# RapidAI/RapidDoc

Hardware: AMD Instinct MI355X
Metric: pages/sec (layout+OCR det/rec) (higher is better)
Workload: dtype f32

## Files before the change

rapiddoc_amd/_lib.py:

```python
from __future__ import annotations

import ctypes as C
from pathlib import Path

_PKG = Path(__file__).resolve().parent
LIB_PATH = _PKG / "librapiddoc_mi355.so"
_lib = None

SYMBOLS = {
    "rd_version": (C.c_char_p, []),
    "rd_create": (C.c_void_p, [C.c_int, C.c_char_p]),
    "rd_create_error": (C.c_char_p, []),
    "rd_destroy": (None, [C.c_void_p]),
    "rd_last_error": (C.c_char_p, [C.c_void_p]),
    "rd_load_weights": (C.c_int, [C.c_void_p, C.c_void_p, C.c_size_t]),
    "rd_query_workspace": (C.c_int, [C.c_void_p, C.c_int, C.c_int, C.c_int, C.c_int, C.POINTER(C.c_size_t)]),
    "rd_det_forward": (C.c_int, [C.c_void_p, C.c_void_p, C.c_int, C.c_int, C.c_int, C.c_void_p, C.c_void_p, C.c_size_t, C.c_void_p]),
    "rd_det_forward_ex": (C.c_int, [C.c_void_p, C.c_void_p, C.c_int, C.c_int, C.c_int, C.c_void_p, C.c_int, C.c_void_p, C.c_void_p, C.c_size_t, C.c_void_p]),
    "rd_rec_forward": (C.c_int, [C.c_void_p, C.c_void_p, C.c_int, C.c_int, C.c_void_p, C.c_void_p, C.c_void_p, C.c_int, C.c_void_p, C.c_size_t, C.c_void_p]),
    "rd_rec_num_classes": (C.c_int, [C.c_void_p]),
    "rd_rec_token_dim": (C.c_int, [C.c_void_p]),
    "rd_rec_backbone_forward": (C.c_int, [C.c_void_p, C.c_void_p, C.c_int, C.c_int, C.c_void_p, C.c_void_p, C.c_size_t, C.c_void_p]),
    "rd_rec_backbone_forward_lines": (C.c_int, [C.c_void_p, C.c_void_p, C.c_int, C.c_int, C.c_void_p, C.c_void_p, C.c_void_p, C.c_size_t, C.c_void_p]),
    "rd_rec_tail_forward": (C.c_int, [C.c_void_p, C.c_void_p, C.c_int, C.c_int, C.c_int, C.c_void_p, C.c_void_p, C.c_void_p, C.c_void_p,
# ... 28 lines not shown
                                     C.c_int, C.c_void_p, C.c_size_t, C.c_void_p, C.c_int, C.c_void_p, C.c_void_p]),
    "rd_rec_chunk_cost": (C.c_double, [C.c_int, C.c_int, C.c_int]),
    "rd_rec_plan_chunks": (C.c_int, [C.c_void_p, C.c_int, C.c_int, C.c_int, C.c_int, C.c_int, C.c_void_p, C.c_int, C.c_void_p]),
    "rd_rec_plan_lines": (C.c_int, [C.c_void_p, C.c_void_p] + [C.c_int] * 9 + [C.c_void_p] * 4 + [C.c_int, C.c_void_p]),
    "rd_text_boxes_order_merge": (C.c_int, [C.c_void_p, C.c_void_p, C.c_int, C.c_int, C.c_void_p, C.c_void_p]),
    "rd_ctc_rows_text": (C.c_int, [C.c_void_p, C.c_int, C.c_int, C.c_void_p, C.c_int64, C.c_void_p, C.c_void_p, C.c_void_p, C.c_void_p]),
    "rd_layout_postprocess": (C.c_int, [C.c_void_p, C.c_int, C.c_int, C.c_int, C.c_int, C.c_void_p, C.c_void_p, C.c_void_p, C.c_void_p]),
    "rd_layout_postprocess_select": (C.c_int, [C.c_void_p, C.c_int, C.c_int, C.c_int, C.c_int, C.c_void_p, C.c_void_p, C.c_void_p, C.c_void_p]),
    "rd_find_external_contours": (C.c_int, [C.c_void_p, C.c_int, C.c_int, C.c_void_p, C.c_int, C.c_void_p, C.c_int, C.c_void_p, C.c_void_p]),
    "rd_find_external_contours_none": (C.c_int, [C.c_void_p, C.c_int, C.c_int, C.c_void_p, C.c_int, C.c_void_p, C.c_int, C.c_void_p, C.c_void_p]),
    "rd_checkbox_workspace": (C.c_size_t, [C.c_int, C.c_int, C.c_int, C.c_int, C.c_int, C.c_void_p]),
    "rd_checkbox_detect_device": (C.c_int, [C.c_int, C.c_void_p, C.c_int, C.c_int, C.c_int, C.c_int, C.c_int, C.c_int, C.c_void_p, C.c_size_t, C.c_void_p,
                                            C.c_void_p, C.c_void_p]),
    "rd_checkbox_finish": (C.c_int, [C.c_void_p, C.c_int, C.c_int, C.c_int, C.c_void_p, C.c_int, C.c_void_p]),
    "rd_region_canvases_workspace": (C.c_size_t, [C.c_int, C.c_int, C.c_int]),
    "rd_region_canvases": (C.c_int, [C.c_int, C.c_void_p, C.c_int, C.c_void_p, C.c_void_p, C.c_int, C.c_int, C.c_void_p, C.c_void_p, C.c_void_p, C.c_size_t,
                                     C.c_void_p]),
    "rd_contour_area": (C.c_double, [C.c_void_p, C.c_int]),
    "rd_arc_length": (C.c_double, [C.c_void_p, C.c_int, C.c_int]),
    "rd_approx_poly_dp": (C.c_int, [C.c_void_p, C.c_int, C.c_double, C.c_int, C.c_void_p, C.c_void_p]),
    "rd_min_area_rect_points": (C.c_int, [C.c_void_p, C.c_int, C.c_void_p]),
    "rd_polygon_area": (C.c_double, [C.c_void_p, C.c_int]),
    "rd_polygon_intersection_area": (C.c_double, [C.c_void_p, C.c_int, C.c_void_p, C.c_int]),
    "rd_fill_poly": (C.c_int, [C.c_void_p, C.c_int, C.c_int, C.c_void_p, C.c_int, C.c_int]),
    "rd_msdeform_attn": (C.c_int, [C.c_int] + [C.c_void_p] * 6 + [C.c_int] * 7 + [C.c_void_p]),
    "rd_topk_rows": (C.c_int, [C.c_int, C.c_void_p, C.c_int, C.c_int, C.c_int, C.c_void_p, C.c_void_p, C.c_void_p]),
    "rd_encoder_layer_workspace": (C.c_size_t, [C.c_int, C.c_int, C.c_int]),
    "rd_encoder_layer": (C.c_int, [C.c_int, C.c_void_p, C.c_void_p] + [C.c_int] * 6 + [C.c_void_p] * 12 + [C.c_float, C.c_void_p, C.c_void_p, C.c_size_t, C.c_void_p]),
    "rd_set_precision": (C.c_int, [C.c_void_p, C.c_char_p]),
    "rd_range_status": (C.c_int, [C.c_void_p, C.c_void_p]),
    "rd_plan_stats": (C.c_int, [C.c_void_p, C.POINTER(C.c_uint64), C.POINTER(C.c_uint64), C.POINTER(C.c_uint64)]),
    "rd_set_profiling": (C.c_int, [C.c_void_p, C.c_int]),
    "rd_profile_json": (C.c_char_p, [C.c_void_p]),
}

_I, _P, _F = C.c_int, C.c_void_p, C.c_float
DEBUG_SYMBOLS = {
    "rd_debug_det_forward_stages": (_I, [_P, _P, _I, _I, _I, _P, _P, _P]),
    "rd_debug_cls_forward_stages": (_I, [_P, _P, _I, _I, _I, _P, _P, _P, _P]),
    "rd_debug_table_decode": (_I, [_P, _P, _I, _I, _I, _P] + [_P] * 7),
    "rd_debug_table_decode_stream": (_I, [_P, _P, _I, _I, _I, _I, _P, _P, _P, _P, _P, _P, _P, _P, _I]),
    "rd_debug_table_encoder_taps": (_I, [_P, _P, _I, _I, _I, _P, _P, _P]),
    "rd_debug_formula_decode": (_I, [_P, _P, _I, _I, _I, _P, C.POINTER(C.c_int32), _P, _P, _P]),
    "rd_debug_formula_decode_stream": (_I, [_P, _P, _I, _I, _I, _I, _P, _P, _P, _P, _P, _P, _P, _I]),
    "rd_debug_resize_aa_coeffs": (_I, [_I, _I, _P, _P, C.c_int64]),
    "rd_debug_resample_coeffs": (_I, [_I, _I, C.c_double, C.c_double, _I, _P, _P, C.c_int64]),
    "rd_debug_region_keep_mask": (_I, [_I, _I, _P, _I, _P]),
    "rd_debug_time_mixer": (_F, [_I] * 4 + [_P] * 6),
    "rd_debug_time_gemm": (_F, [_I] * 5 + [_P] * 6),
    "rd_debug_gemm_h1": (_F, [_I] * 5 + [_P, _I, _P, _P, _P, _I, _P, _I, _P]),
    "rd_debug_seqconv": (_F, [_I] * 8 + [_P, _I, _P, _I, _P, _P, _P, _P, _I, _P]),
    "rd_debug_det_local": (_F, [_I] * 5 + [_P] * 5 + [_F, _P, C.POINTER(C.c_int)]),
    "rd_debug_conv_route": (_I, [_I] * 17 + [_P, _I]),
    "rd_debug_conv_ex": (_F, [_I] * 22 + [_P] * 10 + [C.c_char_p, _P, _I, _P]),
    "rd_debug_conv": (_F, [_I] * 14 + [_P] * 8),
    "rd_debug_stem34": (_F, [_I] * 11 + [_P] * 7),
    "rd_debug_dwconv_ex": (_F, [_I] * 17 + [_P] * 10 + [_I]),
    "rd_debug_dwconv": (_F, [_I] * 8 + [_P] * 8),
    "rd_debug_dw_route": (_I, [_I] * 9 + [_P, _I, _P]),
    "rd_debug_weight_split": (_I, [_P, _I, _I, _P, _P]),
    "rd_debug_lcv3_dw": (_F, [_I] * 9 + [_P] * 8),
    "rd_debug_dw5_strip": (_F, [_I] * 11 + [_P] * 7),
    "rd_debug_mv1e_pool": (_I, [_I] * 4 + [_P] * 3),
    "rd_debug_derived_tensor": (C.c_long, [C.c_char_p, C.c_char_p, C.c_size_t, C.c_char_p, _P, C.c_long]),
    "rd_debug_mbv3_dw": (_F, [_I] * 12 + [_P] * 4),
    "rd_debug_mbv3_block": (_F, [_I] * 14 + [_P] * 8),
    "rd_debug_mbv3_block_ok": (_I, [_I] * 12),
    "rd_debug_mbv3s_dw": (_F, [_I] * 13 + [_P] * 4),
    "rd_debug_mbv3s_block": (_F, [_I] * 15 + [_P] * 12),
    "rd_debug_lcv3_dw_det": (_F, [_I] * 10 + [_P] * 5),
    "rd_debug_lcv3_block": (_F, [_I] * 9 + [_P] * 9),
    "rd_debug_time_ctc": (_F, [_I] * 4 + [_P] * 7 + [_I, _P]),
    "rd_debug_time_checkbox_mask": (_F, [_I] * 4 + [_P, _P]),
    "rd_debug_attention": (_I, [_I] * 4 + [_F, _P, _P, _P, _I, _P]),
    "rd_debug_vit_attention": (_I, [_I] * 4 + [_F, _P, _P]),
    "rd_debug_attention_limits": (_I, [_I, _P, _P]),
    "rd_debug_layernorm": (_I, [_I, _I, _P, _I, _P, _I, _P, _P, _F]),
    "rd_debug_se_chain": (_I, [_I] * 7 + [_F] + [_I] * 3 + [_P] * 9),
    "rd_debug_maxpool2x2s1": (_I, [_I] * 6 + [_P] * 2),
    "rd_debug_avgpool3x2": (_I, [_I] * 6 + [_P] * 3),
    "rd_debug_mask_cols": (_I, [_I] * 5 + [_P, _P, _I]),
    "rd_debug_upsample": (_I, [_I] * 8 + [_P] * 2),
    "rd_debug_add": (_I, [_I] * 5 + [_P] * 3),
    "rd_debug_det_head_tail": (_I, [_I] * 4 + [_P] * 6),
    "rd_debug_ctc_head": (_I, [_I] * 3 + [_P, _I] + [_P] * 6 + [_I, _P, _P]),
    "rd_debug_dec_gemv": (_I, [_I] * 4 + [_P] * 7),
    "rd_debug_dec_attention": (_I, [_I] * 4 + [_P, _P, _I, C.c_longlong] + [_P] * 5 + [_P, _I, _P, _P, _I, _P, _I]),
    "rd_debug_dec_select": (_I, [_I, _P, _I, _I, _I, _P, _I, _P, _I, _I] + [_P] * 6),
}


class NativeLibraryError(RuntimeError):
    pass


def load():
    global _lib
    if _lib is not None:
        return _lib
    if not LIB_PATH.exists():
        raise NativeLibraryError(
            f"{LIB_PATH} is missing - build it with `python -m rapiddoc_amd.build` (hipcc, gfx950). "
            "rapiddoc_amd has no CPU fallback.")
    import torch
    lib = C.CDLL(str(LIB_PATH))
    for name, (res, args) in {**SYMBOLS, **DEBUG_SYMBOLS}.items():
        fn = getattr(lib, name)
        fn.restype = res
        fn.argtypes = args
    _lib = lib
    return lib
```

rapiddoc_amd/csrc/api_debug.cpp:

```cpp
#include <algorithm>
#include <cstring>
#include <functional>
#include <string>
#include <vector>

#include "api_handle.h"
#include "builder_util.h"
#include "region_geom.h"

extern "C" {

static float rd_debug_time(int iters, const std::function<void()>& launch, const std::function<void()>& after_first = nullptr) {
    hipEvent_t e0, e1;
    (void)hipEventCreate(&e0); (void)hipEventCreate(&e1);
    launch();
    if (after_first) after_first();
    (void)hipEventRecord(e0, nullptr);
    for (int i = 0; i < iters; ++i) launch();
    (void)hipEventRecord(e1, nullptr);
    (void)hipEventSynchronize(e1);
    float ms = 0.f;
    (void)hipEventElapsedTime(&ms, e0, e1);
    (void)hipEventDestroy(e0); (void)hipEventDestroy(e1);
    return iters > 0 ? ms / iters : 0.f;
// ... 763 lines not shown
    const bool ok = hipDeviceSynchronize() == hipSuccess && hipGetLastError() == hipSuccess;
    if (range_out) *range_out = flag ? (int)*flag : 0;
    if (flag) (void)hipHostFree(flag);
    return ok ? 0 : -1;
}

int rd_debug_attention(int B, int T, int heads, int hd, float scale, float* qkv, float* o, const int32_t* seg, int route, int* range_out) {
    if (range_out) *range_out = 0;
    if (B <= 0 || T <= 0 || heads <= 0 || !(hd == 15 || hd == 16 || hd == 32) || route < 0 || route > 2) return -1;
    if (route == 2 && !rd::attention_h3_applies(1, hd)) return -1;
    unsigned* flag = debug_flag_new();
    if (!flag) return -1;
    if (route == 0) rd::launch_attention(qkv, o, B, T, heads, hd, scale, nullptr, seg, flag);
    else if (route == 1) rd::launch_attention_valu(qkv, o, B, T, heads, hd, scale, nullptr, seg);
    else rd::launch_attention_h3(qkv, o, B, T, heads, hd, scale, nullptr, seg, flag);
    return debug_finish(flag, range_out);
}
int rd_debug_vit_attention(int B, int T, int heads, int hd, float scale, float* qkv, float* o) {
    if (B <= 0 || B > 65535 || heads <= 0 || heads > 65535 || !qkv || !o || !rd::vit_attention_applies(T, hd)) return -1;
    rd::launch_vit_attention(qkv, o, B, T, heads, scale, nullptr);
    return debug_finish(nullptr, nullptr);
}
int rd_debug_attention_limits(int hd, int* h3_max_t, int* valu_lds_keys) {
    if (!(hd == 15 || hd == 16 || hd == 32)) return -1;
    if (h3_max_t) *h3_max_t = rd::attention_h3_applies(1, hd) ? rd::attention_h3_max_t() : 0;
    if (valu_lds_keys) *valu_lds_keys = rd::attention_lds_keys(hd);
    return 0;
}

int rd_debug_layernorm(int M, int C, float* x, int xld, float* y, int yld, float* g, float* b, float eps) {
    if (M <= 0 || C <= 0 || xld < C || yld < C) return -1;
    if (C == 768) {
        if (xld % 4 || yld % 4) return -1;
        rd::launch_layernorm768(x, xld, y, yld, g, b, M, eps, nullptr);
        return debug_finish(nullptr, nullptr);
    }
    if (C > 512) return -1;
    rd::launch_layernorm(x, xld, y, yld, g, b, M, C, eps, nullptr);
    return debug_finish(nullptr, nullptr);
}

int rd_debug_se_chain(int N, int H, int W, int C, int Cr, int chunks, int gate_act, float alpha, int xld, int yld, int fill_partial, float* x,
                      float* w1, float* b1, float* w2, float* b2, const int32_t* line_w, float* partial, float* gate_out, float* y) {
    if (N <= 0 || H <= 0 || W <= 0 || !rd::se_fc_shape_ok(C) || Cr <= 0 || Cr > 4096 || chunks <= 0) return -1;
    if (!w1 || !b1 || !w2 || !b2 || !partial || !gate_out || (fill_partial && line_w)) return -1;
    if ((fill_partial || y) && (!x || xld < C || xld % 4 != 0)) return -1;
    if (y && (yld < C || yld % 4 != 0)) return -1;
    const int hw = H * W;
    if (fill_partial) rd::launch_gap_partial(x, xld, N, hw, C, partial, chunks, nullptr);
    rd::SeFcParams f{};
    f.partial = partial; f.chunks = chunks; f.N = N; f.C = C; f.Cr = Cr; f.inv_hw = 1.f / (float)hw;
    f.w1 = w1; f.b1 = b1; f.w2 = w2; f.b2 = b2; f.gate = gate_act; f.scale = gate_out; f.H = H;
    if (line_w) { f.line_w = line_w; f.line_w_stride = 1; }
    rd::launch_se_fc(f, nullptr);
    if (y) rd::launch_scale_channels(x, xld, y, yld, gate_out, alpha, N, hw, C, nullptr);
    return debug_finish(nullptr, nullptr);
}

int rd_debug_maxpool2x2s1(int N, int H, int W, int C, int xld, int yld, float* x, float* y) {
    if (N <= 0 || H <= 0 || W <= 0 || C <= 0 || C % 4 || !x || !y || xld < C || xld % 4 || yld < C || yld % 4) return -1;
    rd::launch_maxpool2x2s1(x, xld, y, yld, N, H, W, C, nullptr);
    return debug_finish(nullptr, nullptr);
}
int rd_debug_avgpool3x2(int N, int H, int W, int C, int xld, int yld, float* x, float* y, const int32_t* line_tab) {
    if (N <= 0 || H < 3 || W < 2 || C <= 0 || C % 4 || !x || !y || xld < C || xld % 4 || yld < C || yld % 4 || (line_tab && H / 3 != 1)) return -1;
    rd::launch_avgpool3x2(x, xld, y, yld, N, H, W, C, nullptr, line_tab);
    return debug_finish(nullptr, nullptr);
}
int rd_debug_mask_cols(int N, int H, int W, int C, int yld, float* y, const int32_t* line_w, int stride) {
    if (N <= 0 || H <= 0 || W <= 0 || C <= 0 || C % 4 || !y || yld < C || yld % 4 || !line_w || stride < 1) return -1;
    rd::launch_mask_cols(y, yld, N, H, W, C, line_w, stride, nullptr);
    return debug_finish(nullptr, nullptr);
}
int rd_debug_upsample(int N, int H, int W, int C, int f, int accumulate, int xld, int yld, float* x, float* y) {
    if (N <= 0 || H <= 0 || W <= 0 || C <= 0 || C % 4 || f < 1 || H % f || W % f || !x || !y || xld < C || xld % 4 || yld < C || yld % 4) return -1;
    rd::launch_upsample(x, xld, y, yld, N, H, W, C, f, accumulate, nullptr);
    return debug_finish(nullptr, nullptr);
}
int rd_debug_add(int M, int C, int ald, int bld, int yld, float* a, float* b, float* y) {
    if (M <= 0 || C <= 0 || C % 4 || !a || !b || !y || ald < C || ald % 4 || bld < C || bld % 4 || yld < C || yld % 4) return -1;
    rd::launch_add(a, ald, b, bld, y, yld, M, C, nullptr);
    return debug_finish(nullptr, nullptr);
}

int rd_debug_det_head_tail(int N, int H, int W, int xld, float* x, float* w1, float* b1, float* w2, float* b2, float* y) {
    constexpr int kC = 24;
    if (N <= 0 || H <= 0 || W <= 0 || !x || !w1 || !b1 || !w2 || !b2 || !y || xld < kC || xld % 4 || !rd::det_head_tail_supported(kC, kC, 1)) return -1;
    std::vector<float> h1((size_t)kC * kC * 4), hb1(kC), h2((size_t)kC * 4), hb2(1);
    if (hipMemcpy(h1.data(), w1, h1.size() * 4, hipMemcpyDeviceToHost) != hipSuccess || hipMemcpy(hb1.data(), b1, hb1.size() * 4, hipMemcpyDeviceToHost) != hipSuccess ||
        hipMemcpy(h2.data(), w2, h2.size() * 4, hipMemcpyDeviceToHost) != hipSuccess || hipMemcpy(hb2.data(), b2, 4, hipMemcpyDeviceToHost) != hipSuccess)
        return -1;
    const std::vector<float> one(kC, 1.f), zero(kC, 0.f);
    std::vector<float> wa, ba, wb;
    rd::pack_det_head_tail(h1.data(), hb1.data(), h2.data(), kC, kC, one.data(), zero.data(), wa, ba, wb);
    std::vector<float> img(wa);
    img.insert(img.end(), ba.begin(), ba.end());
    img.insert(img.end(), wb.begin(), wb.end());
    img.push_back(hb2[0]);
    float* d = nullptr;
    if (hipMalloc((void**)&d, img.size() * 4) != hipSuccess) return -1;
    (void)hipMemcpy(d, img.data(), img.size() * 4, hipMemcpyHostToDevice);
    rd::launch_det_head_tail(x, xld, N, H, W, d, d + wa.size(), d + wa.size() + ba.size(), d + wa.size() + ba.size() + wb.size(), y, nullptr);
    const int rc = debug_finish(nullptr, nullptr);
    (void)hipFree(d);
    return rc;
}

int rd_debug_ctc_head(int M, int K, int Ccls, float* x, int xld, float* wp, void* wh, void* wl, float* part, int32_t* idx, float* prob,
                      int nsplit_override, int* nsplit_out, int* range_out) {
    if (range_out) *range_out = 0;
    if (M <= 0 || Ccls <= 0 || K <= 0 || K >= 128 || K % 4 || xld < K || xld % 4 || nsplit_override > 64 || (wh == nullptr) != (wl == nullptr)) return -1;
    rd::CtcParams p{};
    p.x = x; p.xld = xld; p.w = wp; p.M = M; p.K = K; p.C = Ccls; p.part = part;
    p.nsplit = nsplit_override > 0 ? nsplit_override : rd::ctc_head_nsplit(M, Ccls, wh != nullptr);
    p.idx = idx; p.prob = prob;
    p.wh = (const uint16_t*)wh; p.wl = (const uint16_t*)wl;
    if (nsplit_out) *nsplit_out = p.nsplit;
    unsigned* flag = debug_flag_new();
    if (!flag) return -1;
    p.range_flag = flag;
    rd::launch_ctc_head(p, nullptr);
    return debug_finish(flag, range_out);
}

int rd_debug_dec_gemv(int M, int K, int N, int act, const float* x, const float* w, const float* bias, const float* ln_g, const float* ln_b,
                      const float* res, float* y) {
    return rd::debug_dec_gemv(M, K, N, act, x, w, bias, ln_g, ln_b, res, y);
}
int rd_debug_dec_attention(int route, int self, int B, int T, float* kc, float* vc, int ldkv, long long seq_stride, const float* x,
                           const float* ln_g, const float* ln_b, const float* w, const float* bias, const float* q, int ldq, const float* kcur,
                           const float* vcur, int ldcur, float* out, int ldo) {
    return rd::debug_dec_attention(route, self, B, T, kc, vc, ldkv, seq_stride, x, ln_g, ln_b, w, bias, q, ldq, kcur, vcur, ldcur, out, ldo);
}
int rd_debug_dec_select(int mode, const float* logits, int V, int B, int step, int64_t* ids, int ids_ld, int32_t* unfinished, int n_unfinished,
                        int max_new, const float* emb, const float* pos, const float* g, const float* b, float* x, int32_t* state_out) {
    return rd::debug_dec_select(mode, logits, V, B, step, reinterpret_cast<long long*>(ids), ids_ld, unfinished, n_unfinished, max_new, emb, pos, g,
                                b, x, state_out);
}

}
```

rapiddoc_amd/csrc/kernels_misc.hip:

```cpp
#include <cstdlib>
#include <stdexcept>
#include <string>

#include "rd_device.h"

namespace rd {


__device__ __forceinline__ f32x4 act4(f32x4 v, int act) {
    f32x4 r = {rd_act(v[0], act), rd_act(v[1], act), rd_act(v[2], act), rd_act(v[3], act)};
    return r;
}

static inline int grid_for(long total, int block = 256, int cap = 16384) {
    long g = (total + block - 1) / block;
    if (g < 1) g = 1;
    return (int)(g > cap ? cap : g);
}

__global__ void __launch_bounds__(256) dwconv_kernel(DwParams p) {
    const int c4n = p.C >> 2;
    const long total = (long)p.N * p.OH * p.OW * c4n;
    for (long idx = (long)blockIdx.x * 256 + threadIdx.x; idx < total; idx += (long)gridDim.x * 256) {
        const int c = (int)(idx % c4n) << 2;
// ... 538 lines not shown
}
bool det_head_tail_supported(int cin, int cmid, int cout) { return cin == 24 && cmid == 24 && cout == 1; }
void launch_det_head_tail(const float* x, int xld, int N, int H, int W, const float* w1, const float* b1, const float* w2, const float* b2,
                          float* y, hipStream_t s) {
    const long total = (long)N * H * W;
    hipLaunchKernelGGL((det_head_tail_kernel<24, 24>), dim3((unsigned)((total + 255) / 256)), dim3(256), 0, s, x, xld, N, H, W, w1, b1, w2,
                       b2, y);
}

__global__ void __launch_bounds__(256) upsample_kernel(const float* x, int xld, float* y, int yld, int H, int W, int C,
                                                       int f, int accumulate, long total) {
    const int c4n = C >> 2;
    const int IH = H / f, IW = W / f;
    for (long idx = (long)blockIdx.x * 256 + threadIdx.x; idx < total; idx += (long)gridDim.x * 256) {
        const int c = (int)(idx % c4n) << 2;
        const long pix = idx / c4n;
        const int w = pix % W;
        const int h = (pix / W) % H;
        const int n = pix / ((long)W * H);
        f32x4 v = *reinterpret_cast<const f32x4*>(x + (((size_t)n * IH + h / f) * IW + w / f) * xld + c);
        float* yp = y + (size_t)pix * yld + c;
        if (accumulate) v += *reinterpret_cast<const f32x4*>(yp);
        *reinterpret_cast<f32x4*>(yp) = v;
    }
}
void launch_upsample(const float* x, int xld, float* y, int yld, int N, int H, int W, int C, int f, int accumulate,
                     hipStream_t s) {
    const long total = (long)N * H * W * (C >> 2);
    hipLaunchKernelGGL(upsample_kernel, dim3(grid_for(total)), dim3(256), 0, s, x, xld, y, yld, H, W, C, f, accumulate,
                       total);
}

__global__ void __launch_bounds__(256) add_kernel(const float* a, int ald, const float* b, int bld, float* y, int yld,
                                                  int C, long total) {
    const int c4n = C >> 2;
    for (long idx = (long)blockIdx.x * 256 + threadIdx.x; idx < total; idx += (long)gridDim.x * 256) {
        const int c = (int)(idx % c4n) << 2;
        const long m = idx / c4n;
        const f32x4 v = *reinterpret_cast<const f32x4*>(a + (size_t)m * ald + c) +
                        *reinterpret_cast<const f32x4*>(b + (size_t)m * bld + c);
        *reinterpret_cast<f32x4*>(y + (size_t)m * yld + c) = v;
    }
}
void launch_add(const float* a, int ald, const float* b, int bld, float* y, int yld, int M, int C, hipStream_t s) {
    const long total = (long)M * (C >> 2);
    hipLaunchKernelGGL(add_kernel, dim3(grid_for(total)), dim3(256), 0, s, a, ald, b, bld, y, yld, C, total);
}

__device__ __forceinline__ float wave_sum(float v) {
#pragma unroll
    for (int o = 32; o > 0; o >>= 1) v += __shfl_xor(v, o, 64);
    return v;
}
__device__ __forceinline__ float wave_max(float v) {
#pragma unroll
    for (int o = 32; o > 0; o >>= 1) v = fmaxf(v, __shfl_xor(v, o, 64));
    return v;
}

__global__ void __launch_bounds__(256) layernorm_kernel(const float* x, int xld, float* y, int yld, const float* g,
                                                        const float* b, int M, int C, float eps) {
    const int lane = threadIdx.x & 63;
    const int row = blockIdx.x * 4 + (threadIdx.x >> 6);
    if (row >= M) return;
    const float* xr = x + (size_t)row * xld;
    float v[8];
    float s = 0.f;
    int cnt = 0;
    for (int c = lane; c < C; c += 64) {
        v[cnt] = xr[c];
        s += v[cnt++];
    }
    const float mean = wave_sum(s) / C;
    float q = 0.f;
    for (int i = 0; i < cnt; ++i) {
        const float d = v[i] - mean;
        q += d * d;
    }
    const float rstd = rsqrtf(wave_sum(q) / C + eps);
    float* yr = y + (size_t)row * yld;
    cnt = 0;
    for (int c = lane; c < C; c += 64) yr[c] = (v[cnt++] - mean) * rstd * g[c] + b[c];
}
void launch_layernorm(const float* x, int xld, float* y, int yld, const float* g, const float* b, int M, int C,
                      float eps, hipStream_t s) {
    hipLaunchKernelGGL(layernorm_kernel, dim3((M + 3) / 4), dim3(256), 0, s, x, xld, y, yld, g, b, M, C, eps);
}

template <int HD>
__global__ void __launch_bounds__(256) attention_kernel(const float* qkv, float* o, int T, int heads, float scale, const int32_t* seg,
                                                        int tk_cap, int skip_upto) {
    constexpr int HDP = (HD + 3) / 4 * 4;
    constexpr int NV = HDP / 4;
    extern __shared__ float sm[];
    const int TL = min(T, tk_cap);
    f32x4* Ks = reinterpret_cast<f32x4*>(sm);
    f32x4* Vs = Ks + (size_t)TL * NV;
    const int b = blockIdx.x, h = blockIdx.y;
    const int C = heads * HD;
    size_t tok0 = (size_t)b * T;
    if (seg) {
        tok0 = (size_t)seg[2 * b];
        T = seg[2 * b + 1];
        if (T <= skip_upto) return;
    }
    const float* base = qkv + tok0 * 3 * C;
    auto stage = [&](int k0, int kn, bool with_v) {
        for (int i = threadIdx.x; i < kn * HDP; i += 256) {
            const int t = i / HDP, d = i - t * HDP;
            reinterpret_cast<float*>(Ks)[i] = d < HD ? base[(size_t)(k0 + t) * 3 * C + C + h * HD + d] : 0.f;
            if (with_v) reinterpret_cast<float*>(Vs)[i] = d < HD ? base[(size_t)(k0 + t) * 3 * C + 2 * C + h * HD + d] : 0.f;
        }
    };
    const bool tiled = T > TL;
    if (!tiled) {
        stage(0, T, true);
        __syncthreads();
    }
    const int rounds = (T + 255) / 256;
    for (int r = 0; r < rounds; ++r) {
        const int t = r * 256 + threadIdx.x;
        const bool live = t < T;
        f32x4 q[NV];
        const float* qrow = base + (size_t)min(t, T - 1) * 3 * C + h * HD;
#pragma unroll
        for (int v = 0; v < NV; ++v)
#pragma unroll
            for (int e = 0; e < 4; ++e) q[v][e] = qrow[min(4 * v + e, HD - 1)];
#pragma unroll
        for (int v = 0; v < NV; ++v)
#pragma unroll
            for (int e = 0; e < 4; ++e) q[v][e] = (live && 4 * v + e < HD) ? q[v][e] * scale : 0.f;
        auto dot = [&](int j) {
            float sdot = 0.f;
#pragma unroll
            for (int v = 0; v < NV; ++v) {
                const f32x4 kv = Ks[(size_t)j * NV + v];
#pragma unroll
                for (int e = 0; e < 4; ++e)
                    if (4 * v + e < HD) sdot = fmaf(q[v][e], kv[e], sdot);
            }
            return sdot;
        };
        float mx = -INFINITY;
        if (!tiled) {
            if (live)
                for (int j = 0; j < T; ++j) mx = fmaxf(mx, dot(j));
        } else {
            for (int k0 = 0; k0 < T; k0 += TL) {
                const int kn = min(TL, T - k0);
                __syncthreads();
                stage(k0, kn, false);
                __syncthreads();
                if (live)
                    for (int j = 0; j < kn; ++j) mx = fmaxf(mx, dot(j));
            }
        }
        float l = 0.f;
        f32x4 acc[NV];
#pragma unroll
        for (int v = 0; v < NV; ++v) acc[v] = f32x4{0.f, 0.f, 0.f, 0.f};
        auto accumulate = [&](int kn) {
            for (int j0 = 0; j0 < kn; j0 += 64) {
                const int je = min(kn, j0 + 64);
                float lr = 0.f;
                f32x4 ar[NV];
#pragma unroll
                for (int v = 0; v < NV; ++v) ar[v] = f32x4{0.f, 0.f, 0.f, 0.f};
                for (int j = j0; j < je; ++j) {
// ... 77 lines not shown
    smx[threadIdx.x] = mx;
    smi[threadIdx.x] = mi;
    __syncthreads();
    for (int o = 128; o > 0; o >>= 1) {
        if (threadIdx.x < o) {
            const float a = smx[threadIdx.x], b = smx[threadIdx.x + o];
            const int ia = smi[threadIdx.x], ib = smi[threadIdx.x + o];
            if (b > a || (b == a && ib < ia)) { smx[threadIdx.x] = b; smi[threadIdx.x] = ib; }
        }
        __syncthreads();
    }
    const float gmx = smx[0];
    float s = 0.f;
    for (int c = threadIdx.x; c < C; c += 256) s += __expf(zr[c] - gmx);
    ssum[threadIdx.x] = s;
    __syncthreads();
    for (int o = 128; o > 0; o >>= 1) {
        if (threadIdx.x < o) ssum[threadIdx.x] += ssum[threadIdx.x + o];
        __syncthreads();
    }
    if (threadIdx.x == 0) {
        idx[row] = smi[0];
        prob[row] = 1.f / ssum[0];
    }
}
void launch_rowmax_softmax(const float* logits, int ld, int M, int C, int32_t* idx, float* prob, hipStream_t s) {
    if (M > 0) hipLaunchKernelGGL(rowmax_softmax_kernel, dim3(M), dim3(256), 0, s, logits, ld, M, C, idx, prob);
}

__global__ void __launch_bounds__(256) row_softmax_kernel(const float* z, int ld, float* out, int C, int32_t* idx, float* prob) {
    const int row = blockIdx.x;
    const float* zr = z + (size_t)row * ld;
    float mx = -INFINITY;
    for (int c = threadIdx.x; c < C; c += 256) mx = fmaxf(mx, zr[c]);
    __shared__ float red[4];
    mx = wave_max(mx);
    if ((threadIdx.x & 63) == 0) red[threadIdx.x >> 6] = mx;
    __syncthreads();
    mx = fmaxf(fmaxf(red[0], red[1]), fmaxf(red[2], red[3]));
    __syncthreads();
    float s = 0.f;
    for (int c = threadIdx.x; c < C; c += 256) s += __expf(zr[c] - mx);
    s = wave_sum(s);
    if ((threadIdx.x & 63) == 0) red[threadIdx.x >> 6] = s;
    __syncthreads();
    const float inv = 1.f / (red[0] + red[1] + red[2] + red[3]);
    float* orow = out + (size_t)row * C;
    int first = 0x7fffffff;
    for (int c = threadIdx.x; c < C; c += 256) {
        const float pv = __expf(zr[c] - mx) * inv;
        orow[c] = pv;
        if (pv == inv && c < first) first = c;
    }
    if (idx == nullptr) return;
#pragma unroll
    for (int o = 32; o > 0; o >>= 1) first = min(first, __shfl_xor(first, o, 64));
    __shared__ int redi[4];
    if ((threadIdx.x & 63) == 0) redi[threadIdx.x >> 6] = first;
    __syncthreads();
    if (threadIdx.x == 0) {
        idx[row] = min(min(redi[0], redi[1]), min(redi[2], redi[3]));
        prob[row] = inv;
    }
}
void launch_row_softmax(const float* logits, int ld, float* out, int M, int C, hipStream_t s, int32_t* idx, float* prob) {
    if (M > 0) hipLaunchKernelGGL(row_softmax_kernel, dim3(M), dim3(256), 0, s, logits, ld, out, C, idx, prob);
}

__global__ void __launch_bounds__(256) nhwc_to_nchw_kernel(const float* x, int xld, float* y, int HW, int C) {
    __shared__ float tile[32][33];
    const int n = blockIdx.z;
    const int p0 = blockIdx.x * 32, c0 = blockIdx.y * 32;
    const int tx = threadIdx.x & 31, ty = threadIdx.x >> 5;
    for (int r = ty; r < 32; r += 8) {
        const int pp = p0 + r, c = c0 + tx;
        tile[r][tx] = (pp < HW && c < C) ? x[((size_t)n * HW + pp) * xld + c] : 0.f;
    }
    __syncthreads();
    for (int r = ty; r < 32; r += 8) {
        const int c = c0 + r, pp = p0 + tx;
        if (c < C && pp < HW) y[((size_t)n * C + c) * HW + pp] = tile[tx][r];
    }
}
void launch_nhwc_to_nchw(const float* x, int xld, float* y, int N, int H, int W, int C, hipStream_t s) {
    const int HW = H * W;
    hipLaunchKernelGGL(nhwc_to_nchw_kernel, dim3((HW + 31) / 32, (C + 31) / 32, N), dim3(256), 0, s, x, xld, y, HW, C);
}
__global__ void __launch_bounds__(256) nchw_to_nhwc_kernel(const float* x, float* y, int yld, int HW, int C) {
    __shared__ float tile[32][33];
    const int n = blockIdx.z;
    const int p0 = blockIdx.x * 32, c0 = blockIdx.y * 32;
    const int tx = threadIdx.x & 31, ty = threadIdx.x >> 5;
    for (int r = ty; r < 32; r += 8) {
        const int c = c0 + r, pp = p0 + tx;
        tile[r][tx] = (pp < HW && c < C) ? x[((size_t)n * C + c) * HW + pp] : 0.f;
    }
    __syncthreads();
    for (int r = ty; r < 32; r += 8) {
        const int pp = p0 + r, c = c0 + tx;
        if (c < C && pp < HW) y[((size_t)n * HW + pp) * yld + c] = tile[tx][r];
    }
}
void launch_nchw_to_nhwc(const float* x, float* y, int yld, int N, int C, int H, int W, hipStream_t s) {
    const int HW = H * W;
    hipLaunchKernelGGL(nchw_to_nhwc_kernel, dim3((HW + 31) / 32, (C + 31) / 32, N), dim3(256), 0, s, x, y, yld, HW, C);
}

__global__ void __launch_bounds__(256) crop_batch_kernel(CropBatchParams p) {
    const int i = blockIdx.y;
    const CropDesc d = p.descs[i];
    const long plane = (long)p.OH * p.OWp;
    float* dst = p.dst + (size_t)i * 3 * plane;
    const uint8_t* src = p.pages + (size_t)d.page * p.page_stride;
    const float sx = d.rot90 ? d.crop_h / d.out_w : d.crop_w / d.out_w;
    const float sy = d.rot90 ? d.crop_w / p.OH : d.crop_h / p.OH;
    for (long idx = (long)blockIdx.x * 256 + threadIdx.x; idx < plane; idx += (long)gridDim.x * 256) {
        const int ox = idx % p.OWp, oy = idx / p.OWp;
        float out[3] = {0.f, 0.f, 0.f};
        const bool inside = ox < d.out_w;
        if (inside) {
            float u = (ox + 0.5f) * sx - 0.5f, v = (oy + 0.5f) * sy - 0.5f;
            float cx = u, cy = v;
            if (d.rot90) {
                cx = d.crop_w - 1.f - v;
                cy = u;
            }
            cx = fminf(fmaxf(cx, 0.f), d.crop_w - 1.f);
            cy = fminf(fmaxf(cy, 0.f), d.crop_h - 1.f);
            const float wq = d.m[6] * cx + d.m[7] * cy + d.m[8];
            float px = (d.m[0] * cx + d.m[1] * cy + d.m[2]) / wq;
            float py = (d.m[3] * cx + d.m[4] * cy + d.m[5]) / wq;
            px = fminf(fmaxf(px, 0.f), (float)(p.W - 1));
            py = fminf(fmaxf(py, 0.f), (float)(p.H - 1));
            const int x0 = (int)px, y0 = (int)py;
            const int x1 = min(x0 + 1, p.W - 1), y1 = min(y0 + 1, p.H - 1);
            const float tx = px - x0, ty = py - y0;
            const uint8_t* r0 = src + ((size_t)y0 * p.W) * 3;
            const uint8_t* r1 = src + ((size_t)y1 * p.W) * 3;
#pragma unroll
            for (int c = 0; c < 3; ++c) {
                const float a = r0[x0 * 3 + c], b = r0[x1 * 3 + c], e = r1[x0 * 3 + c], f = r1[x1 * 3 + c];
                out[c] = (a * (1.f - tx) + b * tx) * (1.f - ty) + (e * (1.f - tx) + f * tx) * ty;
            }
        }
#pragma unroll
        for (int c = 0; c < 3; ++c) {
            const int sc = p.swap_rb ? 2 - c : c;
            dst[(size_t)c * plane + idx] = inside ? (out[sc] * p.scale - p.mean[c]) * p.inv_std[c] : 0.f;
        }
    }
}
void launch_crop_resize_norm_batch(const CropBatchParams& p, hipStream_t s) {
    if (p.n <= 0) return;
    const long plane = (long)p.OH * p.OWp;
    hipLaunchKernelGGL(crop_batch_kernel, dim3(grid_for(plane, 256, 64), p.n), dim3(256), 0, s, p);
}

}
```

rapiddoc_amd/csrc/rd_kernels.h:

```cpp
#pragma once
#include <hip/hip_runtime.h>
#include <cstdint>
#include <cstdlib>
#include <string>
#include <vector>

#include "../../include/rapiddoc_mi355.h"
#include "rd_host.h"

namespace rd {

enum Act : int { ACT_NONE = 0, ACT_RELU = 1, ACT_GELU = 2, ACT_SILU = 3, ACT_SIGMOID = 4, ACT_HSIG = 5, ACT_HSIG_PADDLE = 6 };
enum OutMode : int { OUT_NHWC = 0, OUT_DECONV2X2 = 1 };

struct ConvParams {
    const float* x; int xld;
    int N, H, W, Cin;
    const float* w;
    const uint16_t* wh;
    const uint16_t* wl;
    const float* bias;
    float* y; int yld;
    int OH, OW, Cout;
    int KH, KW, SH, SW, PT, PL;
// ... 210 lines not shown
    const float* x; int xld;
    int N, H, W, C;
    const float* w;
    const float* bias;
    float* prob;
    float* aux;
};
bool cls_tail_launch_ok(const ClsTailParams& p);
bool launch_cls_tail(const ClsTailParams& p, hipStream_t s);
struct ClsBlockParams {
    const float *we, *be, *wd, *bd, *w1, *b1, *w2, *b2, *wl, *bl;
    int k, cin, mid, cout, sh;
    int se, act, shortcut;
    int ms, es_ld;
};
bool cls_block_plan(ClsBlockParams& L, int H, int W);
size_t cls_block_scratch_floats(const ClsBlockParams& L, int H, int W);
bool cls_block_launch_ok(const ClsBlockParams& L, int N, int H, int W, int xld, int yld);
bool launch_cls_block(const ClsBlockParams& L, const float* x, int xld, float* y, int yld, int N, int H, int W, float* scratch, hipStream_t s);
struct ClsLineParams {
    const float* x; int B, H, W;
    const float* w1c; const float* b1c; int c1;
    ClsBlockParams blk[11]; int n_blocks;
    const float* w2c; const float* b2c; int c2;
    const float* wf; const float* bf;
    float* prob; float* aux;
    float* stage_out[4]; int stage_block[4];
    float* scratch;
    size_t act_floats, d_floats, per_wg;
    int max_blocks = 0;
};
bool cls_line_plan(ClsLineParams& p);
size_t cls_line_scratch_floats(const ClsLineParams& p);
int cls_line_grid(int B, int max_blocks);
bool cls_line_launch_ok(const ClsLineParams& p);
bool launch_cls_line(const ClsLineParams& p, hipStream_t s);
struct LineCropDesc;
int launch_line_flip180(const LineCropDesc* descs, int n, const float* prob, float thresh, uint8_t* scratch, int32_t* flipped, hipStream_t s);
bool lcv3_gap_shape_ok(int c);
void launch_lcv3_gap_rows(const float* x, int xld, int N, int H, int W, int C, float* partial, const int32_t* line_w, int stride, hipStream_t s);
void launch_lcv3_pool(const float* x, int xld, float* y, int yld, int N, int H, int W, int C, float post_s, float post_b, hipStream_t s,
                      const int32_t* line_tab = nullptr);

void launch_maxpool2x2s1(const float* x, int xld, float* y, int yld, int N, int H, int W, int C, hipStream_t s);
void launch_avgpool3x2(const float* x, int xld, float* y, int yld, int N, int H, int W, int C, hipStream_t s, const int32_t* line_tab = nullptr);
void launch_mask_cols(float* y, int yld, int N, int H, int W, int C, const int32_t* line_w, int stride, hipStream_t s);

void launch_gap_partial(const float* x, int xld, int N, int HW, int C, float* partial, int chunks, hipStream_t s);
struct SeFcParams {
    const float* partial; int chunks; int N, C, Cr; float inv_hw;
    const float* w1; const float* b1;
    const float* w2; const float* b2;
    int gate;
    float* scale;
    const int32_t* line_w = nullptr; int line_w_stride = 0; int H = 0;
};
bool se_fc_shape_ok(int c);
void launch_se_fc(const SeFcParams& p, hipStream_t s);
bool det_head_tail_supported(int cin, int cmid, int cout);
void launch_det_head_tail(const float* x, int xld, int N, int H, int W, const float* w1, const float* b1, const float* w2, const float* b2,
                          float* y, hipStream_t s);
struct DetLocalParams {
    const float* f; int fld;
    const float* shrink;
    float* y;
    int N, H, W;
    const float* wimg32;
    const uint16_t* wimg16;
    float w_inv;
    const float* b3;
    const float* w1; float b1;
    unsigned* range_flag;
};
void launch_det_local(const DetLocalParams& p, hipStream_t s);
float prepare_det_local_weights(const float* w3_folded, std::vector<float>& img32, std::vector<uint16_t>& img16);
void launch_scale_channels(const float* x, int xld, float* y, int yld, const float* scale, float alpha,
                           int N, int HW, int C, hipStream_t s);

void launch_upsample(const float* x, int xld, float* y, int yld, int N, int H, int W, int C, int f, int accumulate,
                     hipStream_t s);

void launch_layernorm(const float* x, int xld, float* y, int yld, const float* g, const float* b, int M, int C,
                      float eps, hipStream_t s);
int attention_h3_max_t();
bool attention_h3_applies(int T, int hd);
int attention_lds_keys(int hd);
void launch_attention_h3(const float* qkv, float* o, int B, int T, int heads, int hd, float scale, hipStream_t s, const int32_t* seg,
                         unsigned* range_flag = nullptr);
void launch_attention(const float* qkv, float* o, int B, int T, int heads, int hd, float scale, hipStream_t s, const int32_t* seg = nullptr,
                      unsigned* range_flag = nullptr);
void launch_attention_valu(const float* qkv, float* o, int B, int T, int heads, int hd, float scale, hipStream_t s, const int32_t* seg = nullptr);

bool vit_attention_applies(int T, int hd);
void launch_vit_attention(const float* qkv, float* o, int B, int T, int heads, float scale, hipStream_t s);
void launch_vit_patchify(const float* x, float* y, int B, int H, int W, hipStream_t s);
void launch_vit_add_pos(float* x, const float* pos, int B, int T, int C, hipStream_t s);
void launch_layernorm768(const float* x, int xld, float* y, int yld, const float* g, const float* b, int M, float eps, hipStream_t s);

void launch_add(const float* a, int ald, const float* b, int bld, float* y, int yld, int M, int C, hipStream_t s);

void launch_rowmax_softmax(const float* logits, int ld, int M, int C, int32_t* idx, float* prob, hipStream_t s);
void launch_row_softmax(const float* logits, int ld, float* out, int M, int C, hipStream_t s, int32_t* idx = nullptr, float* prob = nullptr);
struct CtcParams {
    const float* x; int xld;
    const float* w;
    const float* bias;
    int M, K, C;
    float* part;
    int nsplit;
    int32_t* idx; float* prob;
    const uint16_t* wh = nullptr; const uint16_t* wl = nullptr;
    unsigned* range_flag = nullptr;
};
void launch_ctc_head(const CtcParams& p, hipStream_t s);
int ctc_head_nsplit(int M, int C, bool split_fp16);

void launch_nhwc_to_nchw(const float* x, int xld, float* y, int N, int H, int W, int C, hipStream_t s);
void launch_nchw_to_nhwc(const float* x, float* y, int yld, int N, int C, int H, int W, hipStream_t s);

struct PreprocParams {
    const uint8_t* src; int H, W;
    float* dst; int OH, OW;
    float mean[3], inv_std[3]; float scale;
    int interp;
    int swap_rb;
    int batch = 1;
    size_t src_stride = 0, dst_stride = 0;
};
void launch_preproc_resize_norm(const PreprocParams& p, hipStream_t s);

int resize_aa_coeffs(int in, int out, std::vector<int32_t>& bounds, std::vector<int32_t>& kk);
int resample_coeffs(int filter, int in, double box0, double box1, int out, std::vector<int32_t>& bounds, std::vector<int32_t>& kk);
void formula_preproc_plan(int w, int h, rd_formula_plan* plan);
int launch_formula_margin_boxes(int device, const rd_formula_crop* descs_dev, int n, int32_t* boxes_dev, hipStream_t s, std::string& err);
int launch_formula_preproc_batch(int device, const rd_formula_crop* descs, const int32_t* boxes, int n, float* out, uint8_t* out_u8, hipStream_t s,
                                 std::string& err);
int launch_resize_aa_norm(int device, const uint8_t* src, int H, int W, int OH, int OW, const float mean[3], const float std[3], int swap_rb,
                          float* out, uint8_t* out_u8, hipStream_t s, std::string& err);

struct CropDesc {
    int32_t page;
    int32_t out_w;
    float crop_w, crop_h;
    float m[9];
    int32_t rot90;
    int32_t pad_;
};
struct CropBatchParams {
    const uint8_t* pages; int H, W; size_t page_stride;
    const CropDesc* descs; int n;
    float* dst; int OH, OWp;
    float mean[3], inv_std[3]; float scale; int swap_rb;
};
void launch_crop_resize_norm_batch(const CropBatchParams& p, hipStream_t s);

struct LineCropDesc {
    int32_t page;
    int32_t out_w;
    int32_t crop_w, crop_h;
    int32_t rot90;
    int32_t scratch_off;
    double m[9];
};
struct LineCropParams {
    const uint8_t* pages; int H, W; size_t page_stride;
    const LineCropDesc* descs; int n;
    uint8_t* scratch; long max_crop_pixels;
    float* dst; int OH, OWp;
    int swap_rb;
};
int launch_line_crops(const LineCropParams& p, hipStream_t s);
int launch_line_warp(const LineCropParams& p, hipStream_t s);
int launch_line_resize_norm(const LineCropParams& p, hipStream_t s);
int launch_db_scores(const float* prob, int B, int H, int W, const void* cand, const int32_t* n_cand, int max_cand, double* scores, hipStream_t s);
size_t checkbox_workspace_bytes(int P, int H, int W, int max_runs, int max_cand, size_t* offsets);
int launch_checkbox_detect(int device, const uint8_t* pages, int P, int H, int W, int bgr, int max_runs, int max_cand, void* ws, size_t ws_bytes,
                           rd_checkbox_page* hdr, rd_checkbox_cand* cands, hipStream_t s, std::string& err);
void launch_checkbox_bin(const uint8_t* pages, int P, int H, int W, int bgr, uint64_t* bin, hipStream_t s);
int checkbox_finish(const rd_checkbox_cand* cands, int n, int H, int W, rd_checkbox_box* out, int max_out, int32_t* n_out, std::string& err);
size_t region_canvases_workspace_bytes(int n, int gh, int gw);
int launch_region_canvases(int device, const rd_region_desc* descs, int n, const int32_t* pts, const int32_t* boxes, int gh, int gw, uint8_t* canv,
                           uint8_t* det, void* ws, size_t ws_bytes, hipStream_t s, std::string& err);
void find_external_contours(const uint8_t* mask, int h, int w, bool none, std::vector<std::vector<int32_t>>& xy_out);

size_t db_boxes_workspace_bytes(int B, int H, int max_runs, int max_cand);
int launch_db_boxes(const float* prob, int B, int H, int W, const int32_t* src_hw_dev, float thresh, float box_thresh, float unclip_ratio,
                    int dilate, int max_cand, int max_runs, void* ws, size_t ws_bytes, void* out_boxes, int max_out, int32_t* n_out_dev,
                    hipStream_t s);
int launch_ctc_collapse(const int32_t* idx, const float* prob, int B, int T, const int32_t* seg, const uint8_t* ctab, int max_len, int n_classes,
                        uint8_t* out, int row_bytes, uint16_t* kept_cols, float* kept_conf, hipStream_t s);

}

namespace rd {
void split_weights_h3(const float* w, int rows, int K, std::vector<uint16_t>& hi, std::vector<uint16_t>& lo);
struct MixerParams {
    const float* x; int xld;
    float* y; int yld;
    int M, HW, C;
    const float* gate;
// ... 27 lines not shown
```

Baseline: 362.9.

## Add multi-row layernorm and 64x64 vectorized NHWC-to-NCHW transpose kernels

```diff
diff --git a/rapiddoc_amd/_lib.py b/rapiddoc_amd/_lib.py
--- a/rapiddoc_amd/_lib.py
+++ b/rapiddoc_amd/_lib.py
@@ -134,6 +134,8 @@
     "rd_debug_mask_cols": (_I, [_I] * 5 + [_P, _P, _I]),
     "rd_debug_upsample": (_I, [_I] * 8 + [_P] * 2),
     "rd_debug_add": (_I, [_I] * 5 + [_P] * 3),
+    "rd_debug_to_nchw": (_I, [_I] * 5 + [_P] * 2),
+    "rd_debug_time_glue": (_F, [_I] * 10 + [_P] * 4),
     "rd_debug_det_head_tail": (_I, [_I] * 4 + [_P] * 6),
     "rd_debug_ctc_head": (_I, [_I] * 3 + [_P, _I] + [_P] * 6 + [_I, _P, _P]),
     "rd_debug_dec_gemv": (_I, [_I] * 4 + [_P] * 7),
diff --git a/rapiddoc_amd/csrc/api_debug.cpp b/rapiddoc_amd/csrc/api_debug.cpp
--- a/rapiddoc_amd/csrc/api_debug.cpp
+++ b/rapiddoc_amd/csrc/api_debug.cpp
@@ -869,6 +869,34 @@
     rd::launch_add(a, ald, b, bld, y, yld, M, C, nullptr);
     return debug_finish(nullptr, nullptr);
 }
+int rd_debug_to_nchw(int N, int H, int W, int C, int xld, float* x, float* y) {
+    if (N <= 0 || H <= 0 || W <= 0 || C <= 0 || !x || !y || xld < C) return -1;
+    rd::launch_nhwc_to_nchw(x, xld, y, N, H, W, C, nullptr);
+    return debug_finish(nullptr, nullptr);
+}
+float rd_debug_time_glue(int kind, int form, int iters, int nbuf, int N, int H, int W, int C, int xld, int yld, float* x0, float* y0, float* g,
+                         float* b) {
+    if (kind < 0 || kind > 1 || iters <= 0 || nbuf <= 0 || N <= 0 || H <= 0 || W <= 0 || C <= 0 || !x0 || !y0 || xld < C) return -1.f;
+    if (kind == 1 && (C > 512 || yld < C || !g || !b)) return -1.f;
+    const int M = N * H * W;
+    const size_t xn = (size_t)M * xld, yn = (size_t)M * (kind == 0 ? C : yld);
+    auto run = [&](int i) {
+        float *x = x0 + (size_t)(i % nbuf) * xn, *y = y0 + (size_t)(i % nbuf) * yn;
+        if (kind == 0) form ? rd::launch_nhwc_to_nchw_v1(x, xld, y, N, H, W, C, nullptr) : rd::launch_nhwc_to_nchw(x, xld, y, N, H, W, C, nullptr);
+        else form ? rd::launch_layernorm_v1(x, xld, y, yld, g, b, M, C, 1e-6f, nullptr) : rd::launch_layernorm(x, xld, y, yld, g, b, M, C, 1e-6f, nullptr);
+    };
+    hipEvent_t e0, e1;
+    if (hipEventCreate(&e0) != hipSuccess || hipEventCreate(&e1) != hipSuccess) return -1.f;
+    run(0);
+    (void)hipEventRecord(e0, nullptr);
+    for (int i = 0; i < iters; ++i) run(i + 1);
+    (void)hipEventRecord(e1, nullptr);
+    float ms = -1.f;
+    const bool ok = hipEventSynchronize(e1) == hipSuccess && hipEventElapsedTime(&ms, e0, e1) == hipSuccess && hipGetLastError() == hipSuccess;
+    (void)hipEventDestroy(e0);
+    (void)hipEventDestroy(e1);
+    return ok ? ms / iters : -1.f;
+}
 
 int rd_debug_det_head_tail(int N, int H, int W, int xld, float* x, float* w1, float* b1, float* w2, float* b2, float* y) {
     constexpr int kC = 24;
diff --git a/rapiddoc_amd/csrc/kernels_misc.hip b/rapiddoc_amd/csrc/kernels_misc.hip
--- a/rapiddoc_amd/csrc/kernels_misc.hip
+++ b/rapiddoc_amd/csrc/kernels_misc.hip
@@ -644,9 +644,64 @@
     cnt = 0;
     for (int c = lane; c < C; c += 64) yr[c] = (v[cnt++] - mean) * rstd * g[c] + b[c];
 }
+template <int R>
+__global__ void __launch_bounds__(256) layernorm_rows_kernel(const float* x, int xld, float* y, int yld, const float* g,
+                                                             const float* b, int M, int C, float eps) {
+    const int lane = threadIdx.x & 63;
+    const int row0 = (blockIdx.x * 4 + (threadIdx.x >> 6)) * R;
+    if (row0 >= M) return;
+    const bool has0 = lane < C, has1 = lane + 64 < C;
+    const int c0 = has0 ? lane : 0, c1 = has1 ? lane + 64 : 0;
+    float v0[R], v1[R];
+#pragma unroll
+    for (int r = 0; r < R; ++r) {
+        const float* xr = x + (size_t)min(row0 + r, M - 1) * xld;
+        v0[r] = xr[c0];
+        v1[r] = xr[c1];
+    }
+    const float g0 = g[c0], g1 = g[c1], b0 = b[c0], b1 = b[c1];
+    float mean[R], rstd[R];
+#pragma unroll
+    for (int r = 0; r < R; ++r) {
+        float s = 0.f;
+        if (has0) s += v0[r];
+        if (has1) s += v1[r];
+        mean[r] = wave_sum(s) / C;
+    }
+#pragma unroll
+    for (int r = 0; r < R; ++r) {
+        float q = 0.f;
+        if (has0) {
+            const float d = v0[r] - mean[r];
+            q += d * d;
+        }
+        if (has1) {
+            const float d = v1[r] - mean[r];
+            q += d * d;
+        }
+        rstd[r] = rsqrtf(wave_sum(q) / C + eps);
+    }
+#pragma unroll
+    for (int r = 0; r < R; ++r) {
+        if (row0 + r >= M) break;
+        float* yr = y + (size_t)(row0 + r) * yld;
+        if (has0) yr[lane] = (v0[r] - mean[r]) * rstd[r] * g0 + b0;
+        if (has1) yr[lane + 64] = (v1[r] - mean[r]) * rstd[r] * g1 + b1;
+    }
+}
+static inline bool layernorm_v1() {
+    static const bool on = rd_env_on("RD_LAYERNORM_V1");
+    return on;
+}
+void launch_layernorm_v1(const float* x, int xld, float* y, int yld, const float* g, const float* b, int M, int C,
+                         float eps, hipStream_t s) {
+    hipLaunchKernelGGL(layernorm_kernel, dim3((M + 3) / 4), dim3(256), 0, s, x, xld, y, yld, g, b, M, C, eps);
+}
 void launch_layernorm(const float* x, int xld, float* y, int yld, const float* g, const float* b, int M, int C,
                       float eps, hipStream_t s) {
-    hipLaunchKernelGGL(layernorm_kernel, dim3((M + 3) / 4), dim3(256), 0, s, x, xld, y, yld, g, b, M, C, eps);
+    constexpr int R = 4;
+    if (C > 128 || layernorm_v1()) return launch_layernorm_v1(x, xld, y, yld, g, b, M, C, eps, s);
+    hipLaunchKernelGGL((layernorm_rows_kernel<R>), dim3((M + 4 * R - 1) / (4 * R)), dim3(256), 0, s, x, xld, y, yld, g, b, M, C, eps);
 }
 
 template <int HD>
@@ -890,9 +945,68 @@
         if (c < C && pp < HW) y[((size_t)n * C + c) * HW + pp] = tile[tx][r];
     }
 }
+template <bool VEC>
+__global__ void __launch_bounds__(256) nhwc_to_nchw_tile64_kernel(const float* x, int xld, float* y, int HW, int C, int pt_n, int ct_n,
+                                                                  int ntiles, int per_xcd) {
+    constexpr int LD = 65;
+    __shared__ float tile[64 * LD];
+    const int t = (blockIdx.x & 7) * per_xcd + (blockIdx.x >> 3);
+    if (t >= ntiles) return;
+    const int pt = t % pt_n, ct = (t / pt_n) % ct_n, n = t / (pt_n * ct_n);
+    const int p0 = pt * 64, c0 = ct * 64;
+    const int tid = threadIdx.x;
+    {
+        const int q = tid & 15, r = tid >> 4;
+        const int c = c0 + q * 4 < C ? c0 + q * 4 : 0;
+        f32x4 v[4];
+#pragma unroll
+        for (int k = 0; k < 4; ++k) {
+            const int pp = min(p0 + r + 16 * k, HW - 1);
+            v[k] = *reinterpret_cast<const f32x4*>(x + ((size_t)n * HW + pp) * xld + c);
+        }
+#pragma unroll
+        for (int k = 0; k < 4; ++k)
+#pragma unroll
+            for (int i = 0; i < 4; ++i) tile[(q * 4 + i) * LD + r + 16 * k] = v[k][i];
+    }
+    __syncthreads();
+    float* yb = y + ((size_t)n * C + c0) * HW + p0;
+    if (VEC) {
+        const int j = (tid & 15) * 4, r = tid >> 4;
+#pragma unroll
+        for (int k = 0; k < 4; ++k) {
+            const int cc = r + 16 * k;
+            const float* tp = tile + cc * LD + j;
+            const f32x4 o = {tp[0], tp[1], tp[2], tp[3]};
+            if (c0 + cc < C && p0 + j < HW) *reinterpret_cast<f32x4*>(yb + (size_t)cc * HW + j) = o;
+        }
+    } else {
+        const int lane = tid & 63, w = tid >> 6;
+#pragma unroll
+        for (int k = 0; k < 16; ++k) {
+            const int cc = w + 4 * k;
+            const float o = tile[cc * LD + lane];
+            if (c0 + cc < C && p0 + lane < HW) yb[(size_t)cc * HW + lane] = o;
+        }
+    }
+}
+static inline bool to_nchw_v1() {
+    static const bool on = rd_env_on("RD_TO_NCHW_V1");
+    return on;
+}
+void launch_nhwc_to_nchw_v1(const float* x, int xld, float* y, int N, int H, int W, int C, hipStream_t s) {
+    const int HW = H * W;
+    hipLaunchKernelGGL(nhwc_to_nchw_kernel, dim3((HW + 31) / 32, (C + 31) / 32, N), dim3(256), 0, s, x, xld, y, HW, C);
+}
 void launch_nhwc_to_nchw(const float* x, int xld, float* y, int N, int H, int W, int C, hipStream_t s) {
     const int HW = H * W;
-    hipLaunchKernelGGL(nhwc_to_nchw_kernel, dim3((HW + 31) / 32, (C + 31) / 32, N), dim3(256), 0, s, x, xld, y, HW, C);
+    if (to_nchw_v1() || C % 4 || xld % 4 || ((uintptr_t)x & 15)) return launch_nhwc_to_nchw_v1(x, xld, y, N, H, W, C, s);
+    const int pt_n = (HW + 63) / 64, ct_n = (C + 63) / 64;
+    const int ntiles = N * pt_n * ct_n, per_xcd = (ntiles + 7) / 8;
+    if (HW % 4 == 0 && ((uintptr_t)y & 15) == 0)
+        hipLaunchKernelGGL((nhwc_to_nchw_tile64_kernel<true>), dim3(per_xcd * 8), dim3(256), 0, s, x, xld, y, HW, C, pt_n, ct_n, ntiles, per_xcd);
+    else
+        hipLaunchKernelGGL((nhwc_to_nchw_tile64_kernel<false>), dim3(per_xcd * 8), dim3(256), 0, s, x, xld, y, HW, C, pt_n, ct_n, ntiles, per_xcd);
 }
 __global__ void __launch_bounds__(256) nchw_to_nhwc_kernel(const float* x, float* y, int yld, int HW, int C) {
     __shared__ float tile[32][33];
diff --git a/rapiddoc_amd/csrc/rd_kernels.h b/rapiddoc_amd/csrc/rd_kernels.h
--- a/rapiddoc_amd/csrc/rd_kernels.h
+++ b/rapiddoc_amd/csrc/rd_kernels.h
@@ -316,6 +316,8 @@
 
 void launch_layernorm(const float* x, int xld, float* y, int yld, const float* g, const float* b, int M, int C,
                       float eps, hipStream_t s);
+void launch_layernorm_v1(const float* x, int xld, float* y, int yld, const float* g, const float* b, int M, int C,
+                         float eps, hipStream_t s);
 int attention_h3_max_t();
 bool attention_h3_applies(int T, int hd);
 int attention_lds_keys(int hd);
@@ -350,6 +352,7 @@
 int ctc_head_nsplit(int M, int C, bool split_fp16);
 
 void launch_nhwc_to_nchw(const float* x, int xld, float* y, int N, int H, int W, int C, hipStream_t s);
+void launch_nhwc_to_nchw_v1(const float* x, int xld, float* y, int N, int H, int W, int C, hipStream_t s);
 void launch_nchw_to_nhwc(const float* x, float* y, int yld, int N, int C, int H, int W, hipStream_t s);
 
 struct PreprocParams {
```

After: 367.5, median of 3. No clear change (+1.3%).
